# Brochu/RayTrace-WE-GPU

Measured on AMD Instinct MI355X. Metric: Msamples/sec (pixels x spp) at 1920x1080 spp=100 depth=50, higher is better.
Workload: dtype f32

## Files before the change

### raytrace-we-gpu_amd/csrc/rtx_api.hip

```cpp
#include <hip/hip_runtime.h>

#include <algorithm>
#include <cmath>
#include <cstdio>
#include <cstring>
#include <new>
#include <string>
#include <vector>

#include "../../include/rtx.h"
#include "rtx_internal.h"
#include "rtx_prefilter.h"

namespace {

thread_local std::string g_last_error;

int fail(int code, const std::string &msg) {
    g_last_error = msg;
    return code;
}

int hip_fail(hipError_t e, const char *what) {
    return fail(RTX_ERR_HIP, std::string(what) + ": " + hipGetErrorString(e));
}

// ... 629 lines not shown
    }
    for (uint32_t i = 0; i < n; ++i) {
        cen[i] = make_float4(w->spheres[4 * i + 0], w->spheres[4 * i + 1], w->spheres[4 * i + 2],
                             w->spheres[4 * i + 3]);
        const float t = w->mat_types[i];
        mtype[i] = (t == 0.0f) ? 0 : (t == 1.0f) ? 1 : (t == 2.0f) ? 2 : 3;
        mval[i] = make_float4(w->mat_values[4 * i + 0], w->mat_values[4 * i + 1],
                              w->mat_values[4 * i + 2], w->mat_values[4 * i + 3]);
    }
    CullLayout cl;
    const bool linear = c->scan_mode == RTX_SCAN_LINEAR;
    const bool cull = RTX_CULL && !linear && n_pad > rtx::kScanPfMin;
    if (cull) cl = build_cull(w, pre4, flat_hi > flat_lo, flat_cy);
    rtx::LayerGrid grid{};
    std::vector<unsigned long long> gcell;
    const bool has_grid = RTX_GRID_UPLOAD && !linear && n_pad <= rtx::kScanPfMin && flat_hi > flat_lo &&
                          rtx::build_layer_grid(w->spheres, 8 * flat_lo, std::min(8 * flat_hi, n), grid, gcell);
    RTX_HIP(hipStreamSynchronize(c->stream));
    free_world(c);
    const size_t cap = n ? n : 1;
    RTX_HIP(hipMalloc(&c->d_soa, (n_pad ? 4 * (size_t)n_pad : 4) * sizeof(float)));
    RTX_HIP(hipMalloc(&c->d_pre, (n_pad ? 4 * (size_t)n_pad : 4) * sizeof(float)));
    RTX_HIP(hipMalloc(&c->d_pre4, cap * sizeof(float4)));
    RTX_HIP(hipMalloc(&c->d_cen, cap * sizeof(float4)));
    RTX_HIP(hipMalloc(&c->d_mtype, cap * sizeof(int)));
    RTX_HIP(hipMalloc(&c->d_mval, cap * sizeof(float4)));
    if (n) {
        RTX_HIP(hipMemcpyAsync(c->d_soa, soa.data(), soa.size() * sizeof(float), hipMemcpyHostToDevice, c->stream));
        RTX_HIP(hipMemcpyAsync(c->d_pre, pre.data(), pre.size() * sizeof(float), hipMemcpyHostToDevice, c->stream));
        RTX_HIP(hipMemcpyAsync(c->d_pre4, pre4.data(), n * sizeof(float4), hipMemcpyHostToDevice, c->stream));
        RTX_HIP(hipMemcpyAsync(c->d_cen, cen.data(), n * sizeof(float4), hipMemcpyHostToDevice, c->stream));
        RTX_HIP(hipMemcpyAsync(c->d_mtype, mtype.data(), n * sizeof(int), hipMemcpyHostToDevice, c->stream));
// ... 9 lines not shown
                               c->stream));
        RTX_HIP(hipMemcpyAsync(c->d_cbnd2, cl.bnd2.data(), cl.bnd2.size() * sizeof(float), hipMemcpyHostToDevice,
                               c->stream));
        RTX_HIP(hipMalloc(&c->d_cperm, cl.perm.size() * sizeof(uint32_t)));
        RTX_HIP(hipMalloc(&c->d_ccen, cl.perm.size() * sizeof(float4)));
        std::vector<float4> ccen(cl.perm.size());
        for (size_t p = 0; p < ccen.size(); ++p) ccen[p] = cen[cl.perm[p]];
        RTX_HIP(hipMemcpyAsync(c->d_ccen, ccen.data(), ccen.size() * sizeof(float4), hipMemcpyHostToDevice, c->stream));
        RTX_HIP(hipMemcpyAsync(c->d_cpre, cl.pre.data(), cl.pre.size() * sizeof(float), hipMemcpyHostToDevice, c->stream));
        RTX_HIP(hipMemcpyAsync(c->d_cbnd, cl.bnd.data(), cl.bnd.size() * sizeof(float), hipMemcpyHostToDevice, c->stream));
        RTX_HIP(hipMemcpyAsync(c->d_cperm, cl.perm.data(), cl.perm.size() * sizeof(uint32_t), hipMemcpyHostToDevice,
                               c->stream));
        RTX_HIP(hipStreamSynchronize(c->stream));
        c->n_cpad = (uint32_t)cl.perm.size();
        c->cflat_lo = cl.flat_lo;
    }
    if (has_grid) {
        static_assert(sizeof(rtx::LayerGrid) % 8 == 0, "the cells follow the LayerGrid, 8-byte aligned");
        std::vector<unsigned long long> buf(sizeof(rtx::LayerGrid) / 8 + gcell.size());
        std::memcpy(buf.data(), &grid, sizeof grid);
        std::memcpy(buf.data() + sizeof(rtx::LayerGrid) / 8, gcell.data(), gcell.size() * sizeof(unsigned long long));
        RTX_HIP(hipMalloc(&c->d_grid, buf.size() * sizeof(unsigned long long)));
        RTX_HIP(hipMemcpyAsync(c->d_grid, buf.data(), buf.size() * sizeof(unsigned long long), hipMemcpyHostToDevice,
                               c->stream));
        RTX_HIP(hipStreamSynchronize(c->stream));
    }
    if (c->n != n) c->n_changed = true;
    c->n = n;
    c->n_pad = n_pad;
    c->smag = smag_f;
// ... 1016 lines not shown
```

### raytrace-we-gpu_amd/csrc/rtx_grid.h

```cpp
#pragma once

#include <math.h>
#include <stdint.h>

#include <algorithm>
#include <cmath>
#include <utility>
#include <vector>

#if defined(__HIPCC__)
#define RTX_GD __host__ __device__ __forceinline__
#else
#define RTX_GD static inline
#endif

namespace rtx {

constexpr float kGridOMax = 64.0f;
constexpr double kGridFatCells = 1.0 / 256.0;
constexpr double kGridSlabPad = 1e-3;
#ifndef RTX_GRID_STEPS
#define RTX_GRID_STEPS 48
#endif
#ifndef RTX_GRID_HLOG
// ... 215 lines not shown

template <typename Vec>
inline bool build_layer_grid(const float *sph, uint32_t i_lo, uint32_t i_hi, LayerGrid &G, Vec &cell) {
    const uint32_t m = i_hi - i_lo;
    if (m == 0 || (m + 7) / 8 > 64) return false;
    std::vector<std::pair<uint32_t, uint32_t>> hits;
    if (!build_layer_grid_cells(sph + 4 * (size_t)i_lo, m, kGridMaxCells, G,
                                [&](uint32_t k, uint32_t j) { hits.emplace_back(k, j); }))
        return false;
    G.nblk = (m + 7) / 8;
    cell.assign((size_t)G.nx * G.nz, 0ull);
    for (const auto &h : hits) cell[h.first] |= 1ull << (h.second / 8);
    return true;
}

}
```

### raytrace-we-gpu_amd/csrc/rtx_internal.h

```cpp
#pragma once

#include <hip/hip_runtime.h>
#include <stdint.h>

#include "rtx_grid.h"
#include "rtx_refine_keys.h"
#include "rtx_adaptive.h"

struct rtx_ctx;

namespace rtx {

struct KScene {
    const float *soa;
    const float *pre;
    const float4 *pre4;
    const float4 *cen;
    const int *mtype;
    const float4 *mval;
    uint32_t n, n_pad;
    float smag;
    float flat_cy;
    uint32_t flat_lo, flat_hi;
    const float *cpre;
    const float *cbnd;
    const float *cbnd2;
    const float *cbnd3;
    const float4 *ccen;
    const uint32_t *cperm;
    uint32_t n_cpad, cflat_lo;
    const LayerGrid *grid;
};

#ifndef RTX_CULL
#define RTX_CULL 1
#endif
#ifndef RTX_GRID
#define RTX_GRID 1
#endif
#ifndef RTX_CULL_LEVELS
#define RTX_CULL_LEVELS 3
#endif
constexpr uint32_t kCullAlign = RTX_CULL_LEVELS >= 3 ? 512u : 64u;
#ifndef RTX_CULL_HALF
#define RTX_CULL_HALF 1
#endif
#ifndef RTX_CULL_HALF_SPHERES
#define RTX_CULL_HALF_SPHERES 0
#endif
#ifndef RTX_CULL_BFS
#define RTX_CULL_BFS 1
#endif
#ifndef RTX_SCAN_PF_MIN
// ... 98 lines not shown
    float *ps_scratch;
    size_t ps_floats;
    KTune tune;
    hipStream_t aux;
    hipEvent_t ev_fork, ev_join;
    uint32_t *prom_q;
    uint32_t prom_cap;
    uint32_t epoch;
    uint32_t *cost_map;
    uint32_t carry_spp;
};
constexpr uint32_t kSchedWords = 16;
constexpr uint32_t kBlock = 256;

hipError_t launch_render(const KParams &p, const KSchedule &sched, hipStream_t stream);
struct KAdaptive {
    uint8_t *flags;
    uint32_t *n_active;
    uint32_t *count;
    float *err;
    uint32_t active;
};
hipError_t launch_adaptive_mask(const KAdaptive &a, uint32_t width, uint32_t rows, uint32_t samples, float threshold,
                                uint32_t max_samples, hipStream_t stream);
hipError_t launch_adaptive_mask_rows(const KAdaptive &a, const float *halo, uint32_t width, uint32_t rows_local,
                                     uint32_t height, uint32_t tile_rows, uint32_t part, uint32_t nparts,
                                     uint32_t samples, float threshold, uint32_t max_samples, hipStream_t stream);
hipError_t launch_adaptive_edges(const float *err, uint32_t width, uint32_t rows_local, uint32_t tile_rows,
                                 float *edges, hipStream_t stream);
hipError_t launch_render_adaptive(const KParams &p, const KSchedule &sched, const KAdaptive &a, hipStream_t stream);
// ... 27 lines not shown
```

### raytrace-we-gpu_amd/csrc/rtx_kernels.hip

```cpp
#include <algorithm>
#include <cstdlib>
#include <cstring>
#include <mutex>
#include <type_traits>
#include <vector>

#include "rtx_device_math.h"
#include "rtx_diag.h"
#include "rtx_internal.h"
#include "rtx_prefilter.h"

#if defined(__HIP_DEVICE_COMPILE__) && !defined(__gfx950__)
#error "rtx_kernels.hip targets gfx950 (MI355X) only"
#endif

namespace rtx {

namespace {

constexpr float kTMin = 0.001f;

struct FrameVals {
    f3 org, hor, ver, llc;
    float img_w, img_h;
// ... 422 lines not shown
    const bool cand = live & !(disc < 0.0f);
    const float sq = sqrt_rn(disc);
    const float rn = (-hb - sq) * inv_a;
    const float rf = (-hb + sq) * inv_a;
    const bool fin = fabsf(rn) < inf && fabsf(rf) < inf;
    ok = ok & (!cand | fin);
    const float c = !(rn < t_min) ? rn : rf;
    const uint64_t k = ((uint64_t)__float_as_uint(c) << 32) | (uint32_t) ~(uint32_t)(g + 1);
    const bool acc = cand & !(c < t_min) & (k < key);
    key = acc ? k : key;
}

struct GiIdentity {
    __device__ __forceinline__ uint32_t operator()(uint32_t p) const { return p; }
};
template <typename Ld, typename Gi = GiIdentity, bool kPos = false>
__device__ __forceinline__ bool resolve_pre_t(Ld ld, uint32_t n, const uint32_t *list, uint32_t m, f3 o, f3 d,
                                              float a, float inv_a, float t_min, float &best, int &idx,
                                              uint32_t cap = (uint32_t)kCand, Gi gi = Gi()) {
    bool ok = true;
    uint32_t j = 0;
    uint32_t e = list[threadIdx.x];
    RTX_DIAG_ADD(4, (uint32_t)__popcll(__ballot(m != 0u)));
#if RTX_DIAG_PROF
    {
        uint32_t c = 0;
        for (uint32_t q = 0; q < m; ++q) c += (uint32_t)__popc(list[min(q, cap) * kRB + threadIdx.x] >> 24);
#pragma unroll
        for (int off = 32; off > 0; off >>= 1) c += (uint32_t)__shfl_xor((int)c, off, 64);
        RTX_DIAG_ADD(5, c);
// ... 307 lines not shown
        }
    }
    RTX_DIAG_WALK(R.n, rounds);
    (void)rounds;
    unsigned long long *w = reinterpret_cast<unsigned long long *>(spare + (threadIdx.x & ~63u));
    if (slot == 0u) __hip_atomic_store(w, 0ull, __ATOMIC_RELAXED, __HIP_MEMORY_SCOPE_WORKGROUP);
    __atomic_signal_fence(__ATOMIC_SEQ_CST);
    __hip_atomic_fetch_or(w, (unsigned long long)mine, __ATOMIC_RELAXED, __HIP_MEMORY_SCOPE_WORKGROUP);
    __atomic_signal_fence(__ATOMIC_SEQ_CST);
    const unsigned long long v = __hip_atomic_load(w, __ATOMIC_RELAXED, __HIP_MEMORY_SCOPE_WORKGROUP);
    const uint32_t lo = (uint32_t)__builtin_amdgcn_readfirstlane((int)(uint32_t)v);
    const uint32_t hi = (uint32_t)__builtin_amdgcn_readfirstlane((int)(uint32_t)(v >> 32));
    return ((uint64_t)hi << 32) | lo;
}

template <bool kPF, typename Ld, bool kTile = false, bool kGridOk = true>
__device__ __forceinline__ int hit_world_pre_ld(const KScene &S, Ld ld, f3 o, f3 d, float a, float inv_a,
                                                float t_min, float &best, uint32_t *list, uint32_t *pack = nullptr,
                                                uint32_t start = 0, const float *lds_pr = nullptr,
                                                bool live = true) {
    const cfloat_p pre = (cfloat_p)S.pre;
    const uint32_t nblk = S.n_pad / 8;
    RTX_DIAG_HW_BEGIN();
    LineTest T = line_test_setup(o.x, o.y, o.z, d.x, d.y, d.z, a, S.smag);
    if (!live) {
        T.ux = T.uy = T.uz = T.vy = T.vz = T.nou = T.nov = 0.0f;
        T.thr = __uint_as_float(0x7f800000u);
    }
    uint64_t gm = ~0ull;
    if constexpr (!kPF && kGridOk) {
        if (RTX_GRID && S.grid != nullptr) gm = grid_wave_mask(S, o, d, T, list, list + cand_of<kPF>() * kRB);
    }
    RTX_DIAG_HW(0);
    const float best0 = best;
    int idx = -1;
    bool ok = true;
    uint32_t b0 = nblk ? start % nblk : 0u;
    if (RTX_PACK && kPF && pack) {
        const uint32_t at = __builtin_amdgcn_readfirstlane(*pack);
        b0 = at < nblk ? (at + nblk - kPackLag) % nblk : 0u;
    }
    uint32_t b = b0, end = nblk;
    for (;;) {
        uint32_t cnt;
        b = scan_prefilter<kPF, kTile>(pre, b, end, T, S, list, cnt, pack, lds_pr, gm);
        RTX_DIAG_HW(1);
        ok = resolve_pre_t(ld, S.n, list, cnt, o, d, a, inv_a, t_min, best, idx, cand_of<kPF>()) && ok;
        RTX_DIAG_HW(2);
        if (b < end) continue;
        if (end == nblk && b0 != 0u) {
            b = 0;
            end = b0;
            continue;
        }
        break;
    }
    if (!ok) {
        RTX_DIAG_ADD(3, (uint32_t)__popcll(__ballot(1)));
        best = best0;
        idx = hit_blocks_seq((cfloat_p)S.soa, nblk, 0, o, d, a, inv_a, t_min, best, -1);
    }
    return idx;
}
template <bool kPF, bool kGridOk = true>
__device__ __forceinline__ int hit_world_pre(const KScene &S, f3 o, f3 d, float a, float inv_a,
                                             float t_min, float &best, uint32_t *list, uint32_t *pack = nullptr,
                                             uint32_t start = 0) {
    const float4 *__restrict__ cen = S.cen;
    auto ld = [cen](uint32_t i) { return cen[i]; };
    return hit_world_pre_ld<kPF, decltype(ld), false, kGridOk>(S, ld, o, d, a, inv_a, t_min, best, list, pack, start);
}

constexpr uint32_t kCoopSlots = 32;
constexpr uint32_t kCoopWaveBytes = kCoopSlots * 10 * sizeof(float);
constexpr uint32_t kCoopBytes = (kRB / 64) * kCoopWaveBytes;
constexpr uint32_t kCoopLds = 640;
constexpr uint32_t kCoopPad = 128;
static_assert(kCoopMax <= (int)kCoopSlots, "kCoopMax must be <= 32");
__host__ __device__ constexpr uint32_t coop_npad(uint32_t n) { return (n + kCoopPad - 1u) / kCoopPad * kCoopPad; }
__host__ __device__ constexpr uint32_t coop_lds_bytes(uint32_t n) {
    return coop_npad(n) * 4u * (uint32_t)sizeof(float) + n * (uint32_t)sizeof(float);
}
static_assert(coop_lds_bytes(kCoopLds) <= 12800, "LDS copy of the scene: 5 render blocks per CU");

struct SphLds {
    static constexpr bool kPadded = true;
    const float *pr;
    const float *rad;
    uint32_t n, npairs;
    __device__ __forceinline__ void pair(uint32_t p, f2v &cx, f2v &cy, f2v &cz, f2v &R) const {
        const float4 *q = reinterpret_cast<const float4 *>(pr + 8u * p);
        const float4 a = q[0], b = q[1];
        cx = f2v{a.x, a.y};
        cy = f2v{a.z, a.w};
        cz = f2v{b.x, b.y};
        R = f2v{b.z, b.w};
    }
    __device__ __forceinline__ float4 sphere(uint32_t j) const {
// ... 23 lines not shown
    l.pr = base;
    l.rad = base + 8u * l.npairs;
    if (on) {
        float *pr = base, *rad = base + 8u * l.npairs;
        for (uint32_t i = threadIdx.x; i < 2u * l.npairs; i += nthreads) {
            const float4 c = S.pre4[min(i, S.n - 1u)];
            float *q = pr + 8u * (i >> 1) + (i & 1u);
            q[0] = c.x;
            q[2] = c.y;
            q[4] = c.z;
            q[6] = c.w;
            if (i < S.n) rad[i] = S.cen[i].w;
        }
    }
    return l;
}
__device__ __forceinline__ SphGlobal sph_global(const KScene &S) {
    SphGlobal g;
    g.pre = S.pre;
    g.cen = S.cen;
    g.n = S.n;
    g.npairs = S.n_pad / 2u;
    return g;
}

template <bool kMax>
__device__ __forceinline__ uint32_t group_reduce_u32(uint32_t v, uint32_t lg) {
    auto op = [](uint32_t x, uint32_t y) { return kMax ? max(x, y) : min(x, y); };
    if (lg >= 1u) v = op(v, (uint32_t)__builtin_amdgcn_update_dpp(0, (int)v, 0xB1, 0xF, 0xF, false));
    if (lg >= 2u) v = op(v, (uint32_t)__builtin_amdgcn_update_dpp(0, (int)v, 0x4E, 0xF, 0xF, false));
// ... 1067 lines not shown
constexpr uint32_t kExactTile = RTX_EXACT_TILE;

template <bool kPersist, bool kCost = false, bool kPF = false, bool kLin = false, bool kRefine = false,
          bool kAdapt = false>
__global__ void RTX_RENDER_BOUNDS_T2(kPF, kLin) k_render(const KParams P) {
    static_assert(!kAdapt || (kPersist && kRefine && !kCost), "adaptive: the persistent refine render only");
    constexpr bool kCulled = kPF && RTX_CULL && !kLin;
    extern __shared__ __attribute__((aligned(16))) unsigned char s_mem[];
    uint32_t *list = reinterpret_cast<uint32_t *>(s_mem);
    constexpr uint32_t kLB = list_bytes<kPF>();
    float *coop_ws = reinterpret_cast<float *>(s_mem + kLB) + (threadIdx.x / 64) * (kCoopWaveBytes / 4);
    (void)coop_ws;
    const bool coop_lds = P.scene.n <= kCoopLds;
    const SphLds sl = lds_copy(P.scene, reinterpret_cast<float *>(s_mem + kLB + kCoopBytes), coop_lds);
    const SphGlobal sg = sph_global(P.scene);
    uint32_t *pack = kPF ? reinterpret_cast<uint32_t *>(s_mem + kLB + kCoopBytes) : nullptr;
    const float *pf_tile = kPF && (RTX_PF_LDS || RTX_PF_RING) ? reinterpret_cast<const float *>(s_mem + kLB + kCoopBytes + 16) : nullptr;
    __shared__ uint32_t s_server;
    const bool prom_on = kPersist && !kCost && P.prom != nullptr;
    if (kPF && threadIdx.x == 0) *pack = 0u;
    if (prom_on && threadIdx.x == 0) s_server = 0u;
    if (prom_on && blockIdx.x == 0 && threadIdx.x == 0)
        __hip_atomic_store(&P.prom[3], 1u, __ATOMIC_RELAXED, __HIP_MEMORY_SCOPE_AGENT);
    if (coop_lds || kPF || prom_on) __syncthreads();
    const int last = (int)P.scene.n - 1;
    const Frame F = load_frame(P);
    const uint32_t npix = P.rows_local * P.width;
    const uint32_t qlen = kAdapt ? P.qlen : npix;
    const unsigned long long t_start = P.wave_times ? __builtin_amdgcn_s_memrealtime() : 0ull;
    Lane L;
// ... 92 lines not shown
                D.section(1);
                promoted = shade<kCost, kRefine, kAdapt>(P, F, L, min(hit, last), best, prom_on && exhausted ? P.prom_min : 0u);
            }
        } else if ((RTX_PF_LDS || RTX_PF_RING) && kPF) {
            float best = __uint_as_float(0x7f800000u);
            auto ldc = [&P](uint32_t i) { return P.scene.cen[i]; };
            const int hit = hit_world_pre_ld<kPF, decltype(ldc), true>(P.scene, ldc, L.o, L.d, L.a, L.inv_a, kTMin,
                                                                       best, list, nullptr, 0, pf_tile, L.active);
            D.section(1);
            if (L.active) promoted = shade<kCost, kRefine, kAdapt>(P, F, L, min(hit, last), best, prom_on && exhausted ? P.prom_min : 0u);
        } else if (L.active) {
            float best = __uint_as_float(0x7f800000u);
            const int hit = (!kPF && coop_lds)
                                ? hit_world_pre_ld<kPF>(P.scene, [sl](uint32_t i) { return sl.sphere(i); }, L.o, L.d,
                                                        L.a, L.inv_a, kTMin, best, list, nullptr, 0,
                                                        RTX_SCAN_LDS ? sl.pr : nullptr)
                                : hit_world_pre<kPF>(P.scene, L.o, L.d, L.a, L.inv_a, kTMin, best, list, pack);
            D.section(1);
            promoted = shade<kCost, kRefine, kAdapt>(P, F, L, min(hit, last), best, prom_on && exhausted ? P.prom_min : 0u);
        }
        D.section(2);
        if (prom_on)
            written += (uint32_t)__popcll(was_active & ~__ballot(L.active)) - (uint32_t)__popcll(__ballot(promoted));
        if (kPersist && kCost && P.pre_done) pre_count(P, was_active, L);
    }
    D.finish(P);
    count_segments(P, L.segs);
    if (!kDiagAny && P.wave_times && (threadIdx.x & 63u) == 0u) {
        const uint32_t w = blockIdx.x * (kRB / 64) + threadIdx.x / 64;
        P.wave_times[2 * w] = t_start;
        P.wave_times[2 * w + 1] = __builtin_amdgcn_s_memrealtime();
// ... 527 lines not shown
        acc = acc + mk3(v.x, v.y, v.z);
    }
    output_pixel(P, px0 + po, acc);
}

template <bool kPF, bool kLin = false>
__global__ void RTX_PS_BOUNDS_T(kPF) k_render_ps(const KParams P) {
    constexpr bool kCulled = kPF && RTX_CULL && !kLin;
    extern __shared__ __attribute__((aligned(16))) unsigned char s_mem[];
    uint32_t *list = reinterpret_cast<uint32_t *>(s_mem);
    constexpr uint32_t kLB = list_bytes<kPF>();
    float *coop_ws = reinterpret_cast<float *>(s_mem + kLB) + (threadIdx.x / 64) * (kCoopWaveBytes / 4);
    uint32_t *st = reinterpret_cast<uint32_t *>(s_mem + kLB + kCoopBytes) + (threadIdx.x / 64) * kPsSlots * 4;
    const bool sph_lds = !kPF && P.scene.n <= kCoopLds;
    const SphLds sl = lds_copy(P.scene, reinterpret_cast<float *>(s_mem + kLB + kCoopBytes + kPsStateBytes), sph_lds);
    const SphGlobal sg = sph_global(P.scene);
    const uint32_t lane = threadIdx.x & 63u;
    if (lane < kPsSlots * 4) st[lane] = 0u;
    __syncthreads();
    const int last = (int)P.scene.n - 1;
    const Frame F = load_frame(P);
    const uint32_t npix = P.rows_local * P.width;
    const uint32_t wave = blockIdx.x * (kRB / 64) + threadIdx.x / 64;
    float4 *scr = reinterpret_cast<float4 *>(P.ps_scratch) + (size_t)wave * kPsSlots * P.ps_cap;
    const unsigned long long t_start = P.wave_times ? __builtin_amdgcn_s_memrealtime() : 0ull;
    const unsigned long long c_start = P.wave_times ? __builtin_amdgcn_s_memtime() : 0ull;
    PsLane L;
    L.active = false;
    L.segs = 0;
    uint32_t cur = 0, c_px0 = 0, c_npx = 0, c_total = 0, c_issued = 0;
// ... 42 lines not shown
            bool seq = false;
            hit = kCulled
                      ? hit_world_groups_culled<false>(P.scene, act, L.active, L.o, L.d, L.a, L.inv_a, kTMin, coop_ws,
                                                       best, seq)
                  : sph_lds ? hit_world_groups(P.scene, sl, act, L.active, L.o, L.d, L.a, L.inv_a, kTMin, coop_ws, best,
                                               seq)
                            : hit_world_groups(P.scene, sg, act, L.active, L.o, L.d, L.a, L.inv_a, kTMin, coop_ws, best,
                                               seq);
            if (L.active && seq) {
                best = __uint_as_float(0x7f800000u);
                hit = hit_world_pre<kPF>(P.scene, L.o, L.d, L.a, L.inv_a, kTMin, best, list);
            }
        } else if (L.active) {
            hit = kCulled ? hit_world_culled(P.scene, L.o, L.d, L.a, L.inv_a, kTMin, best, list)
                  : sph_lds ? hit_world_pre_ld<kPF>(P.scene, [sl](uint32_t i) { return sl.sphere(i); }, L.o, L.d, L.a,
                                                    L.inv_a, kTMin, best, list)
                            : hit_world_pre<kPF>(P.scene, L.o, L.d, L.a, L.inv_a, kTMin, best, list);
        }
        if (L.active) {
            L.segs++;
            f3 c = mk3(0.0f, 0.0f, 0.0f);
            const int r = path_segment(P, L, min(hit, last), best, c);
            if (r != kSegContinue) {
                scr[(size_t)L.slot * P.ps_cap + L.sidx] = make_float4(c.x, c.y, c.z, 0.0f);
                atomicAdd(&st[4 * L.slot + 3], 1u);
                L.active = false;
                ended = true;
            }
        }
        if (__ballot(ended) == 0ull) continue;
        uint64_t full = __ballot(lane < (uint32_t)kPsSlots && st[4 * lane + 2] != 0u &&
// ... 144 lines not shown

constexpr uint32_t kDebugCulled = 0xffffffffu;
__global__ void __launch_bounds__(kRB) k_debug_hit_world(const KScene S, const float *rays,
                                                            uint32_t nrays, float t_min,
                                                            float t_max, uint32_t start, float *out) {
    __shared__ uint32_t list[list_bytes<true>() > kListBytes ? list_bytes<true>() / sizeof(uint32_t)
                                                             : kListBytes / sizeof(uint32_t)];
    const uint32_t i = blockIdx.x * kRB + threadIdx.x;
    if (i >= nrays) return;
    const f3 o = mk3(rays[6 * i + 0], rays[6 * i + 1], rays[6 * i + 2]);
    const f3 d = mk3(rays[6 * i + 3], rays[6 * i + 4], rays[6 * i + 5]);
    const float a = dir_len2(d);
    const float inv_a = 1.0f / a;
    float best = t_max;
    const int idx =
        min((start == kDebugCulled && S.cpre)
                ? hit_world_culled(S, o, d, a, inv_a, t_min, best, list)
            : S.n_pad > kScanPfMin ? hit_world_pre<true>(S, o, d, a, inv_a, t_min, best, list, nullptr, start)
                                   : hit_world_pre<false>(S, o, d, a, inv_a, t_min, best, list, nullptr, start),
            (int)S.n - 1);
    debug_record(S, o, d, best, idx, out + 10 * (size_t)i);
}

constexpr uint32_t kDebugCulledCoop = 0xffffff00u;
constexpr uint32_t kDebugCulledCoopLane = 0xfffffe00u;
template <bool kBfs>
__global__ void __launch_bounds__(kRB) k_debug_hit_world_coop(const KScene S, const float *rays, uint32_t nrays,
                                                              float t_min, float t_max, uint32_t q, float *out) {
    __shared__ uint32_t list[list_bytes<true>() / sizeof(uint32_t)];
    __shared__ float ws_all[(kRB / 64) * (kCoopWaveBytes / 4)];
    const uint32_t lane = threadIdx.x & 63u, w = threadIdx.x / 64u;
// ... 10 lines not shown
    bool seq = false;
    int idx = hit_world_groups_culled<kBfs>(S, __ballot(active), active, o, d, a, inv_a, t_min,
                                            ws_all + w * (kCoopWaveBytes / 4), best, seq);
    if (!active) return;
    if (seq) {
        best = t_max;
        idx = hit_world_pre<true>(S, o, d, a, inv_a, t_min, best, list);
    }
    debug_record(S, o, d, best, min(idx, (int)S.n - 1), out + 10 * (size_t)i);
}

__global__ void RTX_RENDER_BOUNDS k_debug_scan_rate(const KParams P, uint32_t reps, unsigned long long *sink) {
    extern __shared__ __attribute__((aligned(16))) unsigned char s_mem[];
    uint32_t *list = reinterpret_cast<uint32_t *>(s_mem);
    const SphLds sl = lds_copy(P.scene, reinterpret_cast<float *>(s_mem + kListBytes + kCoopBytes), true);
    __syncthreads();
    const uint32_t npix = P.rows_local * P.width;
    const uint32_t gid = blockIdx.x * kRB + threadIdx.x;
    const uint32_t px = (uint32_t)(((uint64_t)gid * 7919u) % npix);
    uint32_t x, y;
    lane_pixel(P, px, x, y);
    float seed = pixel_seed(P, x, y, 0);
    f3 o, d;
    start_sample(Frame{}, x, y, seed, o, d);
    const float a = dir_len2(d);
    const float inv_a = 1.0f / a;
    uint32_t acc = 0;
    for (uint32_t r = 0; r < reps; ++r) {
        float best = __uint_as_float(0x7f800000u);
        const int hit = hit_world_pre_ld<false>(P.scene, [sl](uint32_t i) { return sl.sphere(i); }, o, d, a, inv_a,
                                                kTMin, best, list, nullptr, 0, RTX_SCAN_LDS ? sl.pr : nullptr);
        acc += (uint32_t)hit ^ __float_as_uint(best);
    }
#pragma unroll
    for (int off = 32; off > 0; off >>= 1) acc += (uint32_t)__shfl_xor((int)acc, off, 64);
    if ((threadIdx.x & 63u) == 0u) atomicAdd(sink, (unsigned long long)acc);
}

__global__ void __launch_bounds__(kBlock) k_debug_math(int fn, const float *in0, const float *in1,
                                                       uint32_t n, float *out) {
    const uint32_t i = blockIdx.x * kBlock + threadIdx.x;
    if (i >= n) return;
    if (fn == 12 || fn == 13) {
        const f3 p = mk3(in0[3 * i], in0[3 * i + 1], in0[3 * i + 2]);
        const f3 nrm = mk3(in1[6 * i], in1[6 * i + 1], in1[6 * i + 2]);
        const f3 rius = mk3(in1[6 * i + 3], in1[6 * i + 4], in1[6 * i + 5]);
// ... 72 lines not shown
    if (!use_pf(s))
        hipLaunchKernelGGL((k_render<kPersist, kCost, false, false, kRefine>), dim3(blocks), dim3(kRB), lds, stream, a);
    else if (use_lin(s))
        hipLaunchKernelGGL((k_render<kPersist, kCost, true, true, kRefine>), dim3(blocks), dim3(kRB), lds, stream, a);
    else
        hipLaunchKernelGGL((k_render<kPersist, kCost, true, false, kRefine>), dim3(blocks), dim3(kRB), lds, stream, a);
}
template <bool kPersist, bool kCost>
static void launch_kr(const KScene &s, uint32_t blocks, size_t lds, hipStream_t stream, const KParams &a) {
    if (a.chain_out)
        launch_k<kPersist, kCost, true>(s, blocks, lds, stream, a);
    else
        launch_k<kPersist, kCost, false>(s, blocks, lds, stream, a);
}

static size_t render_lds(const KScene &s) {
    return (use_pf(s) ? list_bytes<true>() + 16 + (use_lin(s) ? kPfLdsBytes : 0u) : kListBytes) + kCoopBytes +
           (s.n <= kCoopLds ? (size_t)coop_lds_bytes(s.n) : 0);
}

hipError_t launch_cost(const KParams &p, hipStream_t stream) {
    const uint64_t lanes = (uint64_t)p.rows_local * p.width;
    if (lanes == 0 || p.spp == 0 || p.depth == 0 || !p.cost_out) return hipErrorInvalidValue;
    const size_t lds = render_lds(p.scene);
    hipError_t e = allow_lds(render_fn<false, true>(p.scene), lds);
    if (e != hipSuccess) return e;
    launch_k<false, true>(p.scene, ceil_div(tile_span(p.width, p.rows_local, kExactTile), kRB), lds, stream, p);
    return hipGetLastError();
}

#ifndef RTX_PS_ITEMS
#define RTX_PS_ITEMS 512
#endif
constexpr uint32_t kPsItems = RTX_PS_ITEMS;
#ifndef RTX_PS_BPW
#define RTX_PS_BPW 40
#endif
constexpr uint32_t kPsBatchesPerWave = RTX_PS_BPW;
static size_t ps_lds(const KScene &s) {
    return (use_pf(s) ? list_bytes<true>() : kListBytes) + kCoopBytes + kPsStateBytes +
           (!use_pf(s) && s.n <= kCoopLds ? (size_t)coop_lds_bytes(s.n) : 0);
}
static const void *ps_fn(const KScene &s) {
    return !use_pf(s)   ? (const void *)k_render_ps<false>
           : use_lin(s) ? (const void *)k_render_ps<true, true>
                        : (const void *)k_render_ps<true>;
}
static uint32_t ps_cap_of(uint32_t spp) { return max(kPsItems, spp); }
static uint32_t ps_waves(const KParams &p) {
    const uint64_t items = (uint64_t)p.rows_local * p.width * p.spp;
    const uint32_t blocks = min(ceil_div(items, kRB), resident_blocks(ps_fn(p.scene), ps_lds(p.scene)));
    return blocks * (kRB / 64);
}
size_t ps_scratch_floats(const KParams &p) {
    if (p.rng_mode != 1u || p.spp == 0 || p.depth == 0 || (uint64_t)p.rows_local * p.width == 0) return 0;
    return (size_t)ps_waves(p) * kPsSlots * 4 * ps_cap_of(p.spp);
// ... 372 lines not shown

hipError_t launch_chain_image_counts(const float4 *chain, const uint32_t *count, const uint8_t *skip, float4 *image,
                                     size_t pixels, hipStream_t stream) {
    if (pixels == 0) return hipSuccess;
    const uint32_t blocks = (uint32_t)std::min<uint64_t>(((uint64_t)pixels - 1) / kBlock + 1, kFoldBlocks);
    hipLaunchKernelGGL(k_chain_image_counts, dim3(blocks), dim3(kBlock), 0, stream, chain, count, skip, image,
                       (uint64_t)pixels);
    return hipGetLastError();
}

hipError_t launch_debug_hit_world(const KScene &s, const float *rays, uint32_t nrays, float t_min,
                                  float t_max, uint32_t start_block, float *out, hipStream_t stream) {
    if (nrays == 0) return hipSuccess;
    const uint32_t q = start_block & 0xffu;
    const uint32_t sel = start_block & ~0xffu;
    if ((sel == kDebugCulledCoop || sel == kDebugCulledCoopLane) && q >= 1u && q <= 64u && s.cpre) {
        const uint32_t waves = ceil_div(nrays, q);
        if (sel == kDebugCulledCoop)
            hipLaunchKernelGGL(k_debug_hit_world_coop<true>, dim3(ceil_div(waves, kRB / 64u)), dim3(kRB), 0, stream, s,
                               rays, nrays, t_min, t_max, q, out);
        else
            hipLaunchKernelGGL(k_debug_hit_world_coop<false>, dim3(ceil_div(waves, kRB / 64u)), dim3(kRB), 0, stream,
                               s, rays, nrays, t_min, t_max, q, out);
        return hipGetLastError();
    }
    hipLaunchKernelGGL(k_debug_hit_world, dim3(ceil_div(nrays, kRB)), dim3(kRB), 0, stream, s,
                       rays, nrays, t_min, t_max, start_block, out);
    return hipGetLastError();
}

bool debug_scan_rate_supported(const KParams &p) {
    return p.scene.n <= kCoopLds && !use_pf(p.scene) && (uint64_t)p.rows_local * p.width != 0;
}

hipError_t launch_debug_scan_rate(const KParams &p, uint32_t reps, unsigned long long *sink, uint32_t *waves,
                                  hipStream_t stream) {
    if (!debug_scan_rate_supported(p)) return hipErrorInvalidValue;
    const size_t lds = kListBytes + kCoopBytes + (size_t)coop_lds_bytes(p.scene.n);
    const uint32_t blocks = resident_blocks((const void *)k_debug_scan_rate, lds);
    *waves = blocks * (kRB / 64);
    hipLaunchKernelGGL(k_debug_scan_rate, dim3(blocks), dim3(kRB), lds, stream, p, reps, sink);
    return hipGetLastError();
}

hipError_t launch_debug_math(int fn, const float *in0, const float *in1, uint32_t n, float *out,
                             hipStream_t stream) {
    if (n == 0) return hipSuccess;
    hipLaunchKernelGGL(k_debug_math, dim3(ceil_div(n, kBlock)), dim3(kBlock), 0, stream, fn, in0, in1,
                       n, out);
    return hipGetLastError();
}

}
// ... 1 lines not shown
```

Before: 6458.

## Reorder spheres into spatially coherent blocks with LDS position map

Adds a host-side scene layout that groups the dominant flat layer of spheres and orders it by recursive median splits, so that 8-sphere prefilter blocks are spatially compact and grid cells cover fewer blocks. The permuted prefilter data and the permutation are uploaded, and the kernels scan the permuted layout while mapping candidate positions back to scene indices through a 16-bit map held in LDS. This aims to cut wasted prefilter and resolve work per ray. In exchange it adds a little LDS per block and an extra indirection per candidate, and it disables the RTX_SCAN_LDS path.

```diff
diff --git a/raytrace-we-gpu_amd/csrc/rtx_api.hip b/raytrace-we-gpu_amd/csrc/rtx_api.hip
--- a/raytrace-we-gpu_amd/csrc/rtx_api.hip
+++ b/raytrace-we-gpu_amd/csrc/rtx_api.hip
@@ -10,6 +10,7 @@
 
 #include "../../include/rtx.h"
 #include "rtx_internal.h"
+#include "rtx_layout.h"
 #include "rtx_prefilter.h"
 
 namespace {
@@ -669,8 +670,21 @@
     if (cull) cl = build_cull(w, pre4, flat_hi > flat_lo, flat_cy);
     rtx::LayerGrid grid{};
     std::vector<unsigned long long> gcell;
-    const bool has_grid = RTX_GRID_UPLOAD && !linear && n_pad <= rtx::kScanPfMin && flat_hi > flat_lo &&
-                          rtx::build_layer_grid(w->spheres, 8 * flat_lo, std::min(8 * flat_hi, n), grid, gcell);
+    rtx::SceneLayout lay;
+    if (RTX_LAYOUT && !linear && n != 0 && n_pad <= rtx::kScanPfMin) {
+        lay = rtx::build_scene_layout(w->spheres, n, rtx::kLayoutDefault, RTX_GRID_UPLOAD != 0);
+        if (lay.valid && !rtx::layout_lds_ok(n, (uint32_t)lay.perm.size())) lay = rtx::SceneLayout();
+    }
+    bool has_grid;
+    if (lay.valid) {
+        flat_lo = lay.flat_lo, flat_hi = lay.flat_hi, flat_cy = lay.flat_cy;
+        has_grid = lay.has_grid;
+        grid = lay.grid;
+        gcell.swap(lay.cell);
+    } else {
+        has_grid = RTX_GRID_UPLOAD && !linear && n_pad <= rtx::kScanPfMin && flat_hi > flat_lo &&
+                   rtx::build_layer_grid(w->spheres, 8 * flat_lo, std::min(8 * flat_hi, n), grid, gcell);
+    }
     RTX_HIP(hipStreamSynchronize(c->stream));
     free_world(c);
     const size_t cap = n ? n : 1;
@@ -710,6 +724,16 @@
         RTX_HIP(hipStreamSynchronize(c->stream));
         c->n_cpad = (uint32_t)cl.perm.size();
         c->cflat_lo = cl.flat_lo;
+    }
+    if (lay.valid) {
+        RTX_HIP(hipMalloc(&c->d_cpre, lay.pre.size() * sizeof(float)));
+        RTX_HIP(hipMalloc(&c->d_cperm, lay.perm.size() * sizeof(uint32_t)));
+        RTX_HIP(hipMemcpyAsync(c->d_cpre, lay.pre.data(), lay.pre.size() * sizeof(float), hipMemcpyHostToDevice, c->stream));
+        RTX_HIP(hipMemcpyAsync(c->d_cperm, lay.perm.data(), lay.perm.size() * sizeof(uint32_t), hipMemcpyHostToDevice,
+                               c->stream));
+        RTX_HIP(hipStreamSynchronize(c->stream));
+        c->n_cpad = (uint32_t)lay.perm.size();
+        c->cflat_lo = lay.flat_lo;
     }
     if (has_grid) {
         static_assert(sizeof(rtx::LayerGrid) % 8 == 0, "the cells follow the LayerGrid, 8-byte aligned");
diff --git a/raytrace-we-gpu_amd/csrc/rtx_grid.h b/raytrace-we-gpu_amd/csrc/rtx_grid.h
--- a/raytrace-we-gpu_amd/csrc/rtx_grid.h
+++ b/raytrace-we-gpu_amd/csrc/rtx_grid.h
@@ -253,4 +253,22 @@
     return true;
 }
 
-}
+template <typename Vec>
+inline bool build_layer_grid_pos(const float *sph, const uint32_t *perm, uint32_t p_lo, uint32_t p_hi, LayerGrid &G,
+                                 Vec &cell) {
+    const uint32_t m = p_hi - p_lo;
+    if (m == 0 || (m + 7) / 8 > 64) return false;
+    std::vector<float> lay(4 * (size_t)m);
+    for (uint32_t j = 0; j < m; ++j)
+        for (int k = 0; k < 4; ++k) lay[4 * (size_t)j + k] = sph[4 * (size_t)perm[p_lo + j] + k];
+    std::vector<std::pair<uint32_t, uint32_t>> hits;
+    if (!build_layer_grid_cells(lay.data(), m, kGridMaxCells, G,
+                                [&](uint32_t k, uint32_t j) { hits.emplace_back(k, j); }))
+        return false;
+    G.nblk = (m + 7) / 8;
+    cell.assign((size_t)G.nx * G.nz, 0ull);
+    for (const auto &h : hits) cell[h.first] |= 1ull << (h.second / 8);
+    return true;
+}
+
+}
diff --git a/raytrace-we-gpu_amd/csrc/rtx_internal.h b/raytrace-we-gpu_amd/csrc/rtx_internal.h
--- a/raytrace-we-gpu_amd/csrc/rtx_internal.h
+++ b/raytrace-we-gpu_amd/csrc/rtx_internal.h
@@ -37,6 +37,9 @@
 #endif
 #ifndef RTX_GRID
 #define RTX_GRID 1
+#endif
+#ifndef RTX_LAYOUT
+#define RTX_LAYOUT 1
 #endif
 #ifndef RTX_CULL_LEVELS
 #define RTX_CULL_LEVELS 3
@@ -165,6 +168,7 @@
 constexpr uint32_t kBlock = 256;
 
 hipError_t launch_render(const KParams &p, const KSchedule &sched, hipStream_t stream);
+bool layout_lds_ok(uint32_t n, uint32_t n_lpad);
 struct KAdaptive {
     uint8_t *flags;
     uint32_t *n_active;
diff --git a/raytrace-we-gpu_amd/csrc/rtx_kernels.hip b/raytrace-we-gpu_amd/csrc/rtx_kernels.hip
--- a/raytrace-we-gpu_amd/csrc/rtx_kernels.hip
+++ b/raytrace-we-gpu_amd/csrc/rtx_kernels.hip
@@ -460,6 +460,30 @@
 struct GiIdentity {
     __device__ __forceinline__ uint32_t operator()(uint32_t p) const { return p; }
 };
+#if RTX_LAYOUT && RTX_SCAN_LDS
+static_assert(false, "RTX_SCAN_LDS scans the LDS sphere copy, which is in scene order: build it with -DRTX_LAYOUT=0");
+#endif
+__device__ __forceinline__ bool layout_on(const KScene &S) {
+    return RTX_LAYOUT && S.cpre != nullptr && S.n_pad <= kScanPfMin;
+}
+struct MapGlobal {
+    __device__ __forceinline__ uint32_t at(const uint32_t *gmap, uint32_t p) const { return gmap[p]; }
+};
+struct MapLds {
+    const uint16_t *m;
+    __device__ __forceinline__ uint32_t at(const uint32_t *, uint32_t p) const { return (uint32_t)m[p]; }
+};
+template <typename Map>
+struct GiLayout {
+    Map map;
+    const uint32_t *gmap;
+    uint32_t last;
+    bool on;
+    __device__ __forceinline__ uint32_t operator()(uint32_t p) const {
+        if (!on) return p;
+        return map.at(gmap, min(p, last));
+    }
+};
 template <typename Ld, typename Gi = GiIdentity, bool kPos = false>
 __device__ __forceinline__ bool resolve_pre_t(Ld ld, uint32_t n, const uint32_t *list, uint32_t m, f3 o, f3 d,
                                               float a, float inv_a, float t_min, float &best, int &idx,
@@ -797,13 +821,17 @@
     return ((uint64_t)hi << 32) | lo;
 }
 
-template <bool kPF, typename Ld, bool kTile = false, bool kGridOk = true>
+template <bool kPF, typename Ld, bool kTile = false, bool kGridOk = true, typename Map = MapGlobal>
 __device__ __forceinline__ int hit_world_pre_ld(const KScene &S, Ld ld, f3 o, f3 d, float a, float inv_a,
                                                 float t_min, float &best, uint32_t *list, uint32_t *pack = nullptr,
                                                 uint32_t start = 0, const float *lds_pr = nullptr,
-                                                bool live = true) {
-    const cfloat_p pre = (cfloat_p)S.pre;
-    const uint32_t nblk = S.n_pad / 8;
+                                                bool live = true, Map map = Map()) {
+    constexpr bool kLay = !kPF && kGridOk;
+    bool lay = false;
+    if constexpr (kLay) lay = layout_on(S);
+    const cfloat_p pre = (cfloat_p)(lay ? S.cpre : S.pre);
+    const uint32_t nblk = (lay ? S.n_cpad : S.n_pad) / 8;
+    const GiLayout<Map> gi{map, S.cperm, S.n_cpad - 1u, lay};
     RTX_DIAG_HW_BEGIN();
     LineTest T = line_test_setup(o.x, o.y, o.z, d.x, d.y, d.z, a, S.smag);
     if (!live) {
@@ -828,7 +856,10 @@
         uint32_t cnt;
         b = scan_prefilter<kPF, kTile>(pre, b, end, T, S, list, cnt, pack, lds_pr, gm);
         RTX_DIAG_HW(1);
-        ok = resolve_pre_t(ld, S.n, list, cnt, o, d, a, inv_a, t_min, best, idx, cand_of<kPF>()) && ok;
+        if constexpr (!kLay)
+            ok = resolve_pre_t(ld, S.n, list, cnt, o, d, a, inv_a, t_min, best, idx, cand_of<kPF>()) && ok;
+        else
+            ok = resolve_pre_t(ld, S.n, list, cnt, o, d, a, inv_a, t_min, best, idx, cand_of<kPF>(), gi) && ok;
         RTX_DIAG_HW(2);
         if (b < end) continue;
         if (end == nblk && b0 != 0u) {
@@ -841,7 +872,7 @@
     if (!ok) {
         RTX_DIAG_ADD(3, (uint32_t)__popcll(__ballot(1)));
         best = best0;
-        idx = hit_blocks_seq((cfloat_p)S.soa, nblk, 0, o, d, a, inv_a, t_min, best, -1);
+        idx = hit_blocks_seq((cfloat_p)S.soa, S.n_pad / 8, 0, o, d, a, inv_a, t_min, best, -1);
     }
     return idx;
 }
@@ -865,6 +896,10 @@
     return coop_npad(n) * 4u * (uint32_t)sizeof(float) + n * (uint32_t)sizeof(float);
 }
 static_assert(coop_lds_bytes(kCoopLds) <= 12800, "LDS copy of the scene: 5 render blocks per CU");
+__host__ __device__ constexpr uint32_t layout_lds_bytes(uint32_t n_lpad) { return (2u * n_lpad + 15u) & ~15u; }
+static_assert(coop_lds_bytes(486) + layout_lds_bytes(496) <= 12800,
+              "the RTIOW world's sphere copy and position map: 5 render blocks per CU");
+static_assert(kCoopLds + 16u <= 65536u, "the LDS position map holds scene indices in 16 bits");
 
 struct SphLds {
     static constexpr bool kPadded = true;
@@ -918,6 +953,12 @@
         }
     }
     return l;
+}
+__device__ __forceinline__ MapLds lds_pos_map(const KScene &S, void *base, uint32_t nthreads = kRB) {
+    uint16_t *m = reinterpret_cast<uint16_t *>(base);
+    if (layout_on(S))
+        for (uint32_t p = threadIdx.x; p < S.n_cpad; p += nthreads) m[p] = (uint16_t)S.cperm[p];
+    return MapLds{m};
 }
 __device__ __forceinline__ SphGlobal sph_global(const KScene &S) {
     SphGlobal g;
@@ -2015,6 +2056,8 @@
     const bool coop_lds = P.scene.n <= kCoopLds;
     const SphLds sl = lds_copy(P.scene, reinterpret_cast<float *>(s_mem + kLB + kCoopBytes), coop_lds);
     const SphGlobal sg = sph_global(P.scene);
+    const MapLds lmap = kPF || !coop_lds ? MapLds{nullptr}
+                                         : lds_pos_map(P.scene, s_mem + kLB + kCoopBytes + coop_lds_bytes(P.scene.n));
     uint32_t *pack = kPF ? reinterpret_cast<uint32_t *>(s_mem + kLB + kCoopBytes) : nullptr;
     const float *pf_tile = kPF && (RTX_PF_LDS || RTX_PF_RING) ? reinterpret_cast<const float *>(s_mem + kLB + kCoopBytes + 16) : nullptr;
     __shared__ uint32_t s_server;
@@ -2137,7 +2180,7 @@
             const int hit = (!kPF && coop_lds)
                                 ? hit_world_pre_ld<kPF>(P.scene, [sl](uint32_t i) { return sl.sphere(i); }, L.o, L.d,
                                                         L.a, L.inv_a, kTMin, best, list, nullptr, 0,
-                                                        RTX_SCAN_LDS ? sl.pr : nullptr)
+                                                        RTX_SCAN_LDS ? sl.pr : nullptr, true, lmap)
                                 : hit_world_pre<kPF>(P.scene, L.o, L.d, L.a, L.inv_a, kTMin, best, list, pack);
             D.section(1);
             promoted = shade<kCost, kRefine, kAdapt>(P, F, L, min(hit, last), best, prom_on && exhausted ? P.prom_min : 0u);
@@ -2695,6 +2738,9 @@
     uint32_t *st = reinterpret_cast<uint32_t *>(s_mem + kLB + kCoopBytes) + (threadIdx.x / 64) * kPsSlots * 4;
     const bool sph_lds = !kPF && P.scene.n <= kCoopLds;
     const SphLds sl = lds_copy(P.scene, reinterpret_cast<float *>(s_mem + kLB + kCoopBytes + kPsStateBytes), sph_lds);
+    const MapLds lmap = !sph_lds ? MapLds{nullptr}
+                                 : lds_pos_map(P.scene, s_mem + kLB + kCoopBytes + kPsStateBytes +
+                                                            coop_lds_bytes(P.scene.n));
     const SphGlobal sg = sph_global(P.scene);
     const uint32_t lane = threadIdx.x & 63u;
     if (lane < kPsSlots * 4) st[lane] = 0u;
@@ -2767,7 +2813,7 @@
         } else if (L.active) {
             hit = kCulled ? hit_world_culled(P.scene, L.o, L.d, L.a, L.inv_a, kTMin, best, list)
                   : sph_lds ? hit_world_pre_ld<kPF>(P.scene, [sl](uint32_t i) { return sl.sphere(i); }, L.o, L.d, L.a,
-                                                    L.inv_a, kTMin, best, list)
+                                                    L.inv_a, kTMin, best, list, nullptr, 0, nullptr, true, lmap)
                             : hit_world_pre<kPF>(P.scene, L.o, L.d, L.a, L.inv_a, kTMin, best, list);
         }
         if (L.active) {
@@ -2942,7 +2988,7 @@
     const float inv_a = 1.0f / a;
     float best = t_max;
     const int idx =
-        min((start == kDebugCulled && S.cpre)
+        min((start == kDebugCulled && S.cpre && S.n_pad > kScanPfMin)
                 ? hit_world_culled(S, o, d, a, inv_a, t_min, best, list)
             : S.n_pad > kScanPfMin ? hit_world_pre<true>(S, o, d, a, inv_a, t_min, best, list, nullptr, start)
                                    : hit_world_pre<false>(S, o, d, a, inv_a, t_min, best, list, nullptr, start),
@@ -2983,6 +3029,7 @@
     extern __shared__ __attribute__((aligned(16))) unsigned char s_mem[];
     uint32_t *list = reinterpret_cast<uint32_t *>(s_mem);
     const SphLds sl = lds_copy(P.scene, reinterpret_cast<float *>(s_mem + kListBytes + kCoopBytes), true);
+    const MapLds lmap = lds_pos_map(P.scene, s_mem + kListBytes + kCoopBytes + coop_lds_bytes(P.scene.n));
     __syncthreads();
     const uint32_t npix = P.rows_local * P.width;
     const uint32_t gid = blockIdx.x * kRB + threadIdx.x;
@@ -2998,7 +3045,8 @@
     for (uint32_t r = 0; r < reps; ++r) {
         float best = __uint_as_float(0x7f800000u);
         const int hit = hit_world_pre_ld<false>(P.scene, [sl](uint32_t i) { return sl.sphere(i); }, o, d, a, inv_a,
-                                                kTMin, best, list, nullptr, 0, RTX_SCAN_LDS ? sl.pr : nullptr);
+                                                kTMin, best, list, nullptr, 0, RTX_SCAN_LDS ? sl.pr : nullptr, true,
+                                                lmap);
         acc += (uint32_t)hit ^ __float_as_uint(best);
     }
 #pragma unroll
@@ -3101,9 +3149,15 @@
         launch_k<kPersist, kCost, false>(s, blocks, lds, stream, a);
 }
 
+static size_t scene_map_lds(const KScene &s) {
+    return RTX_LAYOUT && s.n <= kCoopLds && s.cpre != nullptr ? (size_t)layout_lds_bytes(s.n_cpad) : 0;
+}
+bool layout_lds_ok(uint32_t n, uint32_t n_lpad) {
+    return n > kCoopLds || coop_lds_bytes(n) + layout_lds_bytes(n_lpad) <= 12800u;
+}
 static size_t render_lds(const KScene &s) {
     return (use_pf(s) ? list_bytes<true>() + 16 + (use_lin(s) ? kPfLdsBytes : 0u) : kListBytes) + kCoopBytes +
-           (s.n <= kCoopLds ? (size_t)coop_lds_bytes(s.n) : 0);
+           (s.n <= kCoopLds ? (size_t)coop_lds_bytes(s.n) : 0) + scene_map_lds(s);
 }
 
 hipError_t launch_cost(const KParams &p, hipStream_t stream) {
@@ -3126,7 +3180,7 @@
 constexpr uint32_t kPsBatchesPerWave = RTX_PS_BPW;
 static size_t ps_lds(const KScene &s) {
     return (use_pf(s) ? list_bytes<true>() : kListBytes) + kCoopBytes + kPsStateBytes +
-           (!use_pf(s) && s.n <= kCoopLds ? (size_t)coop_lds_bytes(s.n) : 0);
+           (!use_pf(s) && s.n <= kCoopLds ? (size_t)coop_lds_bytes(s.n) : 0) + scene_map_lds(s);
 }
 static const void *ps_fn(const KScene &s) {
     return !use_pf(s)   ? (const void *)k_render_ps<false>
@@ -3529,7 +3583,7 @@
     if (nrays == 0) return hipSuccess;
     const uint32_t q = start_block & 0xffu;
     const uint32_t sel = start_block & ~0xffu;
-    if ((sel == kDebugCulledCoop || sel == kDebugCulledCoopLane) && q >= 1u && q <= 64u && s.cpre) {
+    if ((sel == kDebugCulledCoop || sel == kDebugCulledCoopLane) && q >= 1u && q <= 64u && s.cpre && use_pf(s)) {
         const uint32_t waves = ceil_div(nrays, q);
         if (sel == kDebugCulledCoop)
             hipLaunchKernelGGL(k_debug_hit_world_coop<true>, dim3(ceil_div(waves, kRB / 64u)), dim3(kRB), 0, stream, s,
@@ -3551,7 +3605,7 @@
 hipError_t launch_debug_scan_rate(const KParams &p, uint32_t reps, unsigned long long *sink, uint32_t *waves,
                                   hipStream_t stream) {
     if (!debug_scan_rate_supported(p)) return hipErrorInvalidValue;
-    const size_t lds = kListBytes + kCoopBytes + (size_t)coop_lds_bytes(p.scene.n);
+    const size_t lds = kListBytes + kCoopBytes + (size_t)coop_lds_bytes(p.scene.n) + scene_map_lds(p.scene);
     const uint32_t blocks = resident_blocks((const void *)k_debug_scan_rate, lds);
     *waves = blocks * (kRB / 64);
     hipLaunchKernelGGL(k_debug_scan_rate, dim3(blocks), dim3(kRB), lds, stream, p, reps, sink);
diff --git a/raytrace-we-gpu_amd/csrc/rtx_layout.h b/raytrace-we-gpu_amd/csrc/rtx_layout.h
--- /dev/null
+++ b/raytrace-we-gpu_amd/csrc/rtx_layout.h
@@ -0,0 +1,141 @@
+#pragma once
+
+#include <stdint.h>
+#include <string.h>
+
+#include <algorithm>
+#include <map>
+#include <utility>
+#include <vector>
+
+#include "rtx_grid.h"
+#include "rtx_prefilter.h"
+
+namespace rtx {
+
+constexpr uint32_t kLayoutMinLayer = 16;
+constexpr uint32_t kLayoutMaxLayer = 512;
+
+enum LayoutOrder : int { kLayoutScene = 0, kLayoutMedian = 1, kLayoutTiles = 2 };
+constexpr LayoutOrder kLayoutDefault = kLayoutMedian;
+
+struct SceneLayout {
+    bool valid = false;
+    std::vector<float> pre;
+    std::vector<uint32_t> perm;
+    uint32_t flat_lo = 0, flat_hi = 0;
+    float flat_cy = 0.0f;
+    uint32_t n_layer = 0;
+    bool has_grid = false;
+    LayerGrid grid{};
+    std::vector<unsigned long long> cell;
+};
+
+inline uint32_t layout_bits(float v) {
+    uint32_t b;
+    memcpy(&b, &v, sizeof b);
+    return b;
+}
+
+inline std::vector<uint32_t> layout_find_layer(const float *sph, uint32_t n) {
+    std::map<uint32_t, std::pair<uint32_t, uint32_t>> sets;
+    for (uint32_t i = 0; i < n; ++i) {
+        auto it = sets.find(layout_bits(sph[4 * (size_t)i + 1]));
+        if (it == sets.end())
+            sets.emplace(layout_bits(sph[4 * (size_t)i + 1]), std::make_pair(1u, i));
+        else
+            ++it->second.first;
+    }
+    uint32_t best_cnt = 0, best_first = 0, best_bits = 0;
+    for (const auto &s : sets)
+        if (s.second.first > best_cnt || (s.second.first == best_cnt && s.second.second < best_first))
+            best_cnt = s.second.first, best_first = s.second.second, best_bits = s.first;
+    std::vector<uint32_t> ids;
+    if (best_cnt < kLayoutMinLayer || best_cnt > kLayoutMaxLayer) return ids;
+    for (uint32_t i = 0; i < n; ++i)
+        if (layout_bits(sph[4 * (size_t)i + 1]) == best_bits) ids.push_back(i);
+    return ids;
+}
+
+inline void layout_median_split(const float *sph, std::vector<uint32_t> &ids, size_t lo, size_t hi) {
+    const size_t m = hi - lo;
+    if (m <= 8) {
+        std::sort(ids.begin() + lo, ids.begin() + hi);
+        return;
+    }
+    float xlo = INFINITY, xhi = -INFINITY, zlo = INFINITY, zhi = -INFINITY;
+    for (size_t k = lo; k < hi; ++k) {
+        const float x = sph[4 * (size_t)ids[k]], z = sph[4 * (size_t)ids[k] + 2];
+        xlo = std::min(xlo, x), xhi = std::max(xhi, x), zlo = std::min(zlo, z), zhi = std::max(zhi, z);
+    }
+    const int ax = (zhi - zlo) > (xhi - xlo) ? 2 : 0;
+    std::sort(ids.begin() + lo, ids.begin() + hi, [&](uint32_t a, uint32_t b) {
+        const float ca = sph[4 * (size_t)a + ax], cb = sph[4 * (size_t)b + ax];
+        return ca < cb || (ca == cb && a < b);
+    });
+    const size_t nb = (m + 7) / 8;
+    const size_t mid = lo + 8 * (nb / 2);
+    layout_median_split(sph, ids, lo, mid);
+    layout_median_split(sph, ids, mid, hi);
+}
+
+inline void layout_tiles(const float *sph, std::vector<uint32_t> &ids, uint32_t tx, uint32_t tz) {
+    float xlo = INFINITY, xhi = -INFINITY, zlo = INFINITY, zhi = -INFINITY;
+    for (uint32_t i : ids) {
+        const float x = sph[4 * (size_t)i], z = sph[4 * (size_t)i + 2];
+        xlo = std::min(xlo, x), xhi = std::max(xhi, x), zlo = std::min(zlo, z), zhi = std::max(zhi, z);
+    }
+    const double area = std::max((double)(xhi - xlo) * (double)(zhi - zlo), 1e-30);
+    const double s = std::sqrt(area / (double)ids.size());
+    auto key = [&](uint32_t i) {
+        const long kx = (long)std::floor((sph[4 * (size_t)i] - xlo) / (s * tx));
+        const long kz = (long)std::floor((sph[4 * (size_t)i + 2] - zlo) / (s * tz));
+        return std::make_pair(kx, kz);
+    };
+    std::sort(ids.begin(), ids.end(), [&](uint32_t a, uint32_t b) {
+        const auto ka = key(a), kb = key(b);
+        return ka < kb || (ka == kb && a < b);
+    });
+}
+
+inline void layout_order(const float *sph, std::vector<uint32_t> &ids, LayoutOrder order, uint32_t tx = 4,
+                         uint32_t tz = 2) {
+    if (order == kLayoutMedian)
+        layout_median_split(sph, ids, 0, ids.size());
+    else if (order == kLayoutTiles)
+        layout_tiles(sph, ids, tx, tz);
+}
+
+inline SceneLayout build_scene_layout(const float *sph, uint32_t n, LayoutOrder order = kLayoutDefault,
+                                      bool with_grid = true, uint32_t tx = 4, uint32_t tz = 2) {
+    SceneLayout L;
+    std::vector<uint32_t> layer = layout_find_layer(sph, n);
+    if (layer.empty()) return L;
+    L.n_layer = (uint32_t)layer.size();
+    L.flat_cy = sph[4 * (size_t)layer[0] + 1];
+    std::vector<char> in_layer(n, 0);
+    for (uint32_t i : layer) in_layer[i] = 1;
+    layout_order(sph, layer, order, tx, tz);
+    std::vector<char> pad;
+    for (uint32_t i = 0; i < n; ++i)
+        if (!in_layer[i]) L.perm.push_back(i), pad.push_back(0);
+    while (L.perm.size() % 8) L.perm.push_back(L.perm.back()), pad.push_back(1);
+    L.flat_lo = (uint32_t)(L.perm.size() / 8);
+    for (uint32_t i : layer) L.perm.push_back(i), pad.push_back(0);
+    while (L.perm.size() % 8) L.perm.push_back(L.perm.back()), pad.push_back(1);
+    L.flat_hi = (uint32_t)(L.perm.size() / 8);
+    const size_t np = L.perm.size();
+    L.pre.assign(4 * np, 0.0f);
+    for (size_t p = 0; p < np; ++p) {
+        const float *s = sph + 4 * (size_t)L.perm[p];
+        float *blk = &L.pre[32 * (p / 8)];
+        blk[p % 8] = s[0], blk[8 + p % 8] = s[1], blk[16 + p % 8] = s[2];
+        blk[24 + p % 8] = pad[p] ? -INFINITY : prefilter_R(s[0], s[1], s[2], s[3] * s[3]);
+    }
+    if (with_grid)
+        L.has_grid = build_layer_grid_pos(sph, L.perm.data(), 8 * L.flat_lo, 8 * L.flat_hi, L.grid, L.cell);
+    L.valid = true;
+    return L;
+}
+
+}
```

New measurement: 6731 (median of 6 runs). 1.04x the previous value.
